# codyd51/gypsum

Measured on NVIDIA H100. Metric: IQ Msamples/s through 32-PRN x 41-Doppler acquisition (1 ms non-coherent, 2.046 Msps complex64), higher is better.
Workload: dtype f32

## Files before the change

gypsum_b200/csrc/engine.cu:

```cuda
#include <algorithm>
#include <cstddef>
#include <cstdio>
#include <cstdlib>
#include <cstring>
#include <map>
#include <numeric>
#include <string>
#include <tuple>
#include <utility>
#include <vector>

#include "../../include/gypsum_b200.h"
#include "bits_core.cuh"
#include "kernels.cuh"
#include "fix_core.cuh"
#include "nav_core.cuh"
#include "orbit_core.cuh"

using namespace gb;

static_assert(sizeof(gb200_cell_record) == sizeof(CellRecord), "ABI record and device record must match");

namespace {

thread_local std::string g_create_error;

struct DeviceMemory {
    static cudaError_t alloc(void** p, size_t bytes) { return cudaMalloc(p, bytes); }
    static void free(void* p) { cudaFree(p); }
};
struct PinnedMemory {
    static cudaError_t alloc(void** p, size_t bytes) { return cudaMallocHost(p, bytes); }
    static void free(void* p) { cudaFreeHost(p); }
};

template <class T, class Memory>
struct Buf {
    T* p = nullptr;
    size_t cap = 0;
    Buf() = default;
    Buf(const Buf&) = delete;
    Buf& operator=(const Buf&) = delete;
    Buf(Buf&& o) noexcept : p(std::exchange(o.p, nullptr)), cap(std::exchange(o.cap, 0)) {}
    ~Buf() { release(); }
    cudaError_t ensure(size_t n) {
        if (n <= cap) return cudaSuccess;
        release();
        size_t want = std::max(n, static_cast<size_t>(16));
        cudaError_t e = Memory::alloc(reinterpret_cast<void**>(&p), want * sizeof(T));
        if (e == cudaSuccess) cap = want;
        return e;
    }
    void release() {
        if (p) Memory::free(p);
        p = nullptr;
        cap = 0;
    }
};
template <class T>
using DevBuf = Buf<T, DeviceMemory>;
template <class T>
using PinnedBuf = Buf<T, PinnedMemory>;

constexpr int kL2WindowMb = 16;

int env_int(const char* name, int dflt) {
    const char* v = getenv(name);
    return (v && *v) ? atoi(v) : dflt;
}

}

struct gb200_engine {
    int device = 0, fs = 0, N = 0, s = 0, num_sms = 132;
    cudaStream_t own_stream = nullptr, stream = nullptr;
    DevBuf<float2> tw1, tw2, crep, iq_own, spec, d_replica;
    DevBuf<uint8_t> chips;
    DevBuf<double> d_doppler;
    DevBuf<int> d_ints;
    DevBuf<CellRecord> d_records;
    DevBuf<float> d_profile;
    DevBuf<RefineState> r_state;
    DevBuf<double> r_doppler;
    DevBuf<CellRecord> r_records;
    DevBuf<int> r_ints;
    DevBuf<RefineResult> r_results;
    DevBuf<int> r_cell_prn;
    PinnedBuf<int> rh_cell_prn;
    PinnedBuf<int> rh_ints;
    PinnedBuf<RefineResult> rh_results;
    PinnedBuf<float2> h_iq, h_replica;
    PinnedBuf<CellRecord> h_records;
    PinnedBuf<int> h_ints;
    PinnedBuf<double> h_doubles;
    PinnedBuf<float> h_profile;
    std::vector<double> doppler_cache;
    std::vector<int> prn_cache;
    bool grid_cache_valid = false;
    int n_prn = 0;
    const float2* iq = nullptr;
    int64_t iq_samples = 0;
    int64_t launches = 0;
    size_t spec_budget_bytes = 512u << 20;
    bool timing = false;
    int fused = -1;
    bool fused_configured = false;
    DevBuf<BestRecord> d_best;
    PinnedBuf<BestRecord> h_best;
    struct HostGraph {
        struct Key {
            int n_blocks = 0, M = 0, P = 0, D = 0, kind = 0;
            std::vector<double> dop;
            std::vector<int> prn;
            const void *iq_dev = nullptr, *rec_dev = nullptr, *iq_stage = nullptr, *rec_stage = nullptr, *spec = nullptr;
            const void *d_dop = nullptr, *d_prn = nullptr, *crep = nullptr;
            const void* rec_target = nullptr;
            cudaStream_t stream = nullptr;
            auto ids() const {
                return std::tie(n_blocks, M, P, D, kind, iq_dev, rec_dev, iq_stage, rec_stage, spec, d_dop, d_prn, crep, rec_target,
                                stream);
            }
            bool operator==(const Key& o) const {
                return ids() == o.ids() && dop.size() == o.dop.size() && prn == o.prn &&
                       memcmp(dop.data(), o.dop.data(), sizeof(double) * dop.size()) == 0;
            }
        } key;
        cudaGraphExec_t exec = nullptr;
        int seen = 0;
    } hg;
    std::vector<std::pair<cudaEvent_t, cudaEvent_t>> ev[2];
    size_t ev_used[2] = {0, 0};
    std::string err;

    ~gb200_engine() {
        if (hg.exec) cudaGraphExecDestroy(hg.exec);
        for (auto& pool : ev)
            for (auto& pr : pool) {
                cudaEventDestroy(pr.first);
                cudaEventDestroy(pr.second);
            }
        if (own_stream) cudaStreamDestroy(own_stream);
    }
};

struct TrackerChain {
    struct Output {
        std::vector<int> counts;
        int stride = 0;
        int n_ms = 0;
        bool pending = false;
    };
    Output records;
    Output bits;
// ... 181 lines not shown
        if (stop) cudaEventRecord(stop, e->stream);
    }
};

int pick_rsplit(const gb200_engine* e, int slots, long long n_cells) {
    if (n_cells >= 8LL * e->num_sms * slots) return 1;
    return std::gcd(e->s, slots);
}

size_t unit_floats2(const gb200_engine* e, int M) { return static_cast<size_t>(M) * e->s * 2 * kFft; }

int run_spectra(gb200_engine* e, const float2* iq, int M, const double* dop, int n_doppler, int n_units) {
    SpectraArgs sa{};
    sa.iq = iq;
    sa.doppler = dop;
    sa.spec = e->spec.p;
    sa.tw1 = e->tw1.p;
    sa.tw2 = e->tw2.p;
    sa.block_stride = static_cast<long long>(M) * e->N;
    sa.inv_fs = 1.0 / static_cast<double>(e->fs);
    sa.N = e->N;
    sa.s = e->s;
    sa.M = M;
    sa.n_doppler = n_doppler;
    sa.n_units = n_units;
    GB_LAUNCH(e, 0, launch_doppler_spectra(sa, e->stream));
    return GB200_OK;
}

CorrelateArgs correlate_args(const gb200_engine* e, int M, int kind, int rsplit, CellRecord* records, float* profile) {
    CorrelateArgs ca{};
    ca.spec = e->spec.p;
    ca.crep = e->crep.p;
    ca.tw1 = e->tw1.p;
    ca.tw2 = e->tw2.p;
    ca.records = records;
    ca.profile = profile;
    ca.N = e->N;
    ca.s = e->s;
    ca.M = M;
    ca.kind = kind;
    ca.rsplit = rsplit;
    return ca;
}

int fused_args(gb200_engine* e, int M, FusedArgs* fa) {
    if (!e->fused_configured) {
        GB_CUDA(e, configure_fused_kernel());
        e->fused_configured = true;
    }
    *fa = FusedArgs{};
    fa->iq = e->iq;
    fa->crep = e->crep.p;
    fa->tw1 = e->tw1.p;
    fa->tw2 = e->tw2.p;
    fa->inv_fs = 1.0 / static_cast<double>(e->fs);
    fa->N = e->N;
    fa->M = M;
    return GB200_OK;
}

struct ListPlan {
    std::vector<int> cell_u, cell_out, grp_first, grp_count, grp_prn;
    size_t size() const { return 2 * cell_u.size() + 3 * grp_prn.size(); }
    void write(int* host) const {
        for (const auto* v : {&cell_u, &cell_out, &grp_first, &grp_count, &grp_prn}) host = std::copy(v->begin(), v->end(), host);
// ... 365 lines not shown
    if ((ce = e->tw2.ensure(kFft)) != cudaSuccess) return fail(ce, "cudaMalloc");
    if ((ce = launch_init_tables(e->tw1.p, e->tw2.p, e->stream)) != cudaSuccess) return fail(ce, "init_tables");
    e->launches++;
    if ((ce = cudaStreamSynchronize(e->stream)) != cudaSuccess) return fail(ce, "init_tables sync");
    *out = e;
    return GB200_OK;
}

int gb200_destroy(gb200_engine* e) {
    if (!e) return GB200_OK;
    cudaSetDevice(e->device);
    cudaStreamSynchronize(e->stream);
    delete e;
    return GB200_OK;
}

int gb200_set_stream(gb200_engine* e, void* st) {
    if (!e) return GB200_EINVAL;
    GB_CUDA(e, cudaSetDevice(e->device));
    GB_CUDA(e, cudaStreamSynchronize(e->stream));
    e->stream = st ? static_cast<cudaStream_t>(st) : e->own_stream;
    return GB200_OK;
}

int gb200_set_replicas(gb200_engine* e, const uint8_t* chips, int n_prn) {
    if (!e) return GB200_EINVAL;
    if (!chips || n_prn < 1) GB_FAIL(e, GB200_EINVAL, "need at least one PRN code");
    for (int i = 0; i < n_prn * kChips; ++i)
        if (chips[i] > 1) GB_FAIL(e, GB200_EINVAL, "chips must be 0 or 1");
    GB_CUDA(e, cudaSetDevice(e->device));
    GB_CUDA(e, cudaStreamSynchronize(e->stream));
    GB_CUDA(e, e->chips.ensure(static_cast<size_t>(n_prn) * kChips));
    GB_CUDA(e, e->crep.ensure(static_cast<size_t>(n_prn) * 2 * kFft));
    GB_CUDA(e, cudaMemcpyAsync(e->chips.p, chips, static_cast<size_t>(n_prn) * kChips, cudaMemcpyHostToDevice, e->stream));
    GB_LAUNCH(e, -1, launch_replica_spectra(e->chips.p, n_prn, e->crep.p, e->stream));
    GB_CUDA(e, cudaStreamSynchronize(e->stream));
    e->n_prn = n_prn;
    return GB200_OK;
}

int gb200_upload_iq(gb200_engine* e, const float* iq_host, int64_t n_samples) {
    if (!e) return GB200_EINVAL;
    if (!iq_host || n_samples < 0) GB_FAIL(e, GB200_EINVAL, "bad IQ buffer");
    GB_CUDA(e, cudaSetDevice(e->device));
    GB_CUDA(e, e->iq_own.ensure(static_cast<size_t>(std::max<int64_t>(n_samples, 1))));
    const float2* src = reinterpret_cast<const float2*>(iq_host);
    if (!is_pinned(iq_host)) {
        GB_CUDA(e, cudaStreamSynchronize(e->stream));
        GB_CUDA(e, stage_in(e->h_iq, src, static_cast<size_t>(n_samples)));
    }
    GB_CUDA(e, cudaMemcpyAsync(e->iq_own.p, src, static_cast<size_t>(n_samples) * sizeof(float2), cudaMemcpyHostToDevice,
                               e->stream));
    e->iq = e->iq_own.p;
    e->iq_samples = n_samples;
    return GB200_OK;
}

int gb200_bind_iq_device(gb200_engine* e, const void* iq_device, int64_t n_samples) {
    if (!e) return GB200_EINVAL;
    if (!iq_device || n_samples < 0) GB_FAIL(e, GB200_EINVAL, "bad IQ buffer");
    if (reinterpret_cast<uintptr_t>(iq_device) % 16 != 0) GB_FAIL(e, GB200_EINVAL, "IQ buffer must be 16-byte aligned");
    e->iq = static_cast<const float2*>(iq_device);
    e->iq_samples = n_samples;
    return GB200_OK;
}

int gb200_acquire_grid_device(gb200_engine* e, int n_blocks, int M, const int32_t* prn_idx, int P, const double* dop, int D,
                              int kind, void* out_device) {
// ... 45 lines not shown
                            const double* dop, int D, int kind, gb200_cell_record* out_host) {
    if (!e) return GB200_EINVAL;
    if (!iq_host || !out_host) GB_FAIL(e, GB200_EINVAL, "null buffer");
    GB_TRY(check_grid(e, std::min(n_blocks, M), P, D, prn_idx, dop));
    GB_CUDA(e, cudaSetDevice(e->device));
    const size_t n_iq = static_cast<size_t>(n_blocks) * M * e->N, n_rec = static_cast<size_t>(n_blocks) * P * D;
    const size_t spec_bytes = unit_floats2(e, M) * D * sizeof(float2) * n_blocks;
    if (e->timing || spec_bytes > e->spec_budget_bytes) {
        GB_TRY(gb200_upload_iq(e, iq_host, static_cast<int64_t>(n_iq)));
        return gb200_acquire_grid(e, n_blocks, M, prn_idx, P, dop, D, kind, out_host);
    }
    GB_CUDA(e, cudaStreamSynchronize(e->stream));
    GB_CUDA(e, e->iq_own.ensure(n_iq));
    GB_CUDA(e, e->h_iq.ensure(n_iq));
    GB_CUDA(e, e->d_records.ensure(n_rec));
    GB_CUDA(e, e->h_records.ensure(n_rec));
    const float2* h2d_src = reinterpret_cast<const float2*>(iq_host);
    const bool eager_src = n_iq * sizeof(float2) > (64u << 10) && is_pinned(iq_host);
    if (!eager_src) GB_CUDA(e, stage_in(e->h_iq, h2d_src, n_iq));
    e->iq = e->iq_own.p;
    e->iq_samples = static_cast<int64_t>(n_iq);

    GB_TRY(check_replicas(e));
    GB_TRY(check_prns(e, prn_idx, P));
    GB_TRY(upload_grid_axes(e, prn_idx, P, dop, D));
    const bool direct = n_rec * sizeof(CellRecord) <= (256u << 10);
    void* caller_alias = nullptr;
    const bool to_caller = direct && is_pinned(out_host, &caller_alias) && caller_alias;
    CellRecord* rec_target = to_caller ? static_cast<CellRecord*>(caller_alias) : direct ? e->h_records.p : e->d_records.p;
    auto& g = e->hg;
    auto key = [&] {
        return gb200_engine::HostGraph::Key{n_blocks, M, P, D, kind, {dop, dop + D}, {prn_idx, prn_idx + P},
                                            e->iq_own.p, e->d_records.p, e->h_iq.p, e->h_records.p, e->spec.p,
                                            e->d_doppler.p, e->d_ints.p, e->crep.p, rec_target, e->stream};
    };
    const bool same = g.seen && g.key == key();
    auto enqueue = [&]() -> int {
        GB_CUDA(e, cudaMemcpyAsync(e->iq_own.p, h2d_src, n_iq * sizeof(float2), cudaMemcpyHostToDevice, e->stream));
        GB_TRY(run_grid(e, n_blocks, M, prn_idx, P, dop, D, kind, rec_target));
        if (!direct)
            GB_CUDA(e, cudaMemcpyAsync(e->h_records.p, e->d_records.p, n_rec * sizeof(CellRecord), cudaMemcpyDeviceToHost, e->stream));
        return GB200_OK;
    };
    if (eager_src) {
        GB_TRY(enqueue());
    } else if (same && g.exec) {
        GB_CUDA(e, cudaGraphLaunch(g.exec, e->stream));
        e->launches += 2;
    } else if (same && !g.exec && g.seen == 1) {
        g.seen = 2;
        GB_CUDA(e, cudaStreamBeginCapture(e->stream, cudaStreamCaptureModeThreadLocal));
        int rc = enqueue();
        cudaGraph_t graph = nullptr;
        cudaError_t ce = cudaStreamEndCapture(e->stream, &graph);
        if (rc == GB200_OK && ce == cudaSuccess && graph) ce = cudaGraphInstantiate(&g.exec, graph, 0);
        if (graph) cudaGraphDestroy(graph);
        if (rc != GB200_OK || ce != cudaSuccess || !g.exec) {
            cudaGetLastError();
            g.exec = nullptr;
            GB_TRY(enqueue());
        } else {
            GB_CUDA(e, cudaGraphLaunch(g.exec, e->stream));
        }
    } else {
        if (!same) {
            if (g.exec) cudaGraphExecDestroy(g.exec);
            g.exec = nullptr;
// ... 966 lines not shown
```

gypsum_b200/csrc/kernels.cu:

```cuda
#include "kernels.cuh"
#include "ptx_helpers.cuh"
#include "warp_fft.cuh"

namespace gb {

__global__ void k_init_tables(float2* tw1, float2* tw2) {
    const int t = blockIdx.x * blockDim.x + threadIdx.x;
    if (t >= 1024) return;
    {
        const int k1 = t >> 5, l = t & 31;
        double s, c;
        sincospi(-2.0 * ((l * k1) & 1023) / 1024.0, &s, &c);
        tw1[pidx(k1, l)] = make_float2(static_cast<float>(c), static_cast<float>(s));
    }
    {
        double s, c;
        sincospi(-2.0 * t / 2048.0, &s, &c);
        tw2[zpos(t)] = make_float2(static_cast<float>(c), static_cast<float>(s));
    }
}

__global__ void __launch_bounds__(128) k_replica_spectra(const uint8_t* chips, float2* crep) {
    __shared__ double2 cs[kPad];
    __shared__ uint8_t c[1024];
    const int p = blockIdx.y;
    for (int t = threadIdx.x; t < kPad; t += blockDim.x) {
        double s, co;
        sincospi(2.0 * t / kPad, &s, &co);
        cs[t] = make_double2(co, s);
    }
    for (int t = threadIdx.x; t < kChips; t += blockDim.x) c[t] = chips[p * kChips + t];
    __syncthreads();
    const int g = blockIdx.x * blockDim.x + threadIdx.x;
    double re, im;
    replica_spectrum_bin(c, g, cs, re, im);
    crep[(static_cast<size_t>(p) * 2 + (g & 1)) * kFft + zpos(g >> 1)] = make_float2(static_cast<float>(re), static_cast<float>(im));
}

__host__ __device__ constexpr int spec_warps(int s) { return 2 * s >= 8 ? 8 : 2 * s; }
constexpr int kCarrierTable = 64;

__host__ __device__ constexpr bool spec_alias(int s) { return 2 * s <= 8; }
__host__ __device__ constexpr int spec_f2(int s) {
    return spec_alias(s) ? (s * kFft > spec_warps(s) * kTileF2 ? s * kFft : spec_warps(s) * kTileF2)
                         : s * kFft + spec_warps(s) * kTileF2;
}

template <int S>
__global__ void __launch_bounds__(spec_warps(S) * 32, S == 2 ? 4 : 1) k_doppler_spectra(const SpectraArgs a) {
    constexpr int kSpecWarps = spec_warps(S);
    constexpr int kSpecThreads = kSpecWarps * 32;
    extern __shared__ __align__(16) float2 smem[];
    float2* ypoly = smem;
    float2* tiles = spec_alias(S) ? smem : smem + S * kFft;
    float2* coarse = smem + spec_f2(S);

    const int unit = blockIdx.x / a.M, i = blockIdx.x % a.M;
    const int b = unit / a.n_doppler, d = unit % a.n_doppler;
    const double f = a.doppler[d];
    if (isnan(f)) return;
    const float2* __restrict__ src = a.iq + static_cast<size_t>(b) * a.block_stride + static_cast<size_t>(i) * a.N;
    const int tid = threadIdx.x;

    constexpr int kIter = (kChips * S + kSpecThreads - 1) / kSpecThreads;
    constexpr int kBatch = kIter < 16 ? kIter : 16;
    float2 v[kBatch];
#pragma unroll
    for (int k = 0; k < kBatch; ++k) {
        const int n = tid + k * kSpecThreads;
// ... 210 lines not shown
                    pair_barrier(pair);
                }
                Peak t;
                float fsum;
                thread_peak16(acc, lane, h, a.s, r, t, fsum);
                t.sum = static_cast<double>(fsum);
                peak_merge(pk, t);
                if (PROFILE && KIND != kKindCoherent) {
#pragma unroll
                    for (int jj = 0; jj < 16; ++jj) {
                        const int q = lane + 32 * (16 * h + jj);
                        if (q < kChips) a.profile[a.s * q + r] = acc[jj];
                    }
                }
            }
            warp_reduce_peak(pk);
            if (KIND == kKindCoherent) warp_reduce_probe(pr_re, pr_im);
            if (lane == 0) store_partial(partial + warp, pk, pr_re, pr_im);
        }
        if (a.rsplit == 1) {
            if (active) pair_barrier(pair);
        } else {
            __syncthreads();
        }
        if (active && (pair % a.rsplit) == 0 && h == 0 && lane == 0) {
            float pre, pim;
            const Peak m = merge_partials(partial + warp, 2 * a.rsplit, pre, pim);
            write_record(a.records + out, m, pre, pim);
        }
        if (a.rsplit != 1) __syncthreads();
    }
}

template <int NW, bool SINGLE_MS>
__global__ void __launch_bounds__(NW * 32, 1) k_correlate_w2048(const CorrelateArgs a) {
    extern __shared__ __align__(16) float2 smem[];
    constexpr int kCrepOdd = kFft;
    float2* crep_s = smem;
    float2* tw1_s = crep_s + 2 * kFft;
    float2* tw1o_s = tw1_s + kFft;
    float2* tiles = tw1o_s + kFft / 2;
    PeakPartial* partial = reinterpret_cast<PeakPartial*>(tiles + NW * kTile64F2);
    uint64_t* mbar = reinterpret_cast<uint64_t*>(partial + NW);

    const int warp = threadIdx.x >> 5, lane = threadIdx.x & 31;
    float2* tile = tiles + warp * kTile64F2;

    uint32_t parity = 0;
    if (threadIdx.x == 0) mbar_init(mbar, 1);
    __syncthreads();
    if (threadIdx.x == 0) {
        mbar_expect_tx(mbar, kFft * sizeof(float2));
        bulk_g2s(tw1_s, a.tw1, kFft * sizeof(float2), mbar);
    }
    mbar_wait(mbar, parity);
    parity ^= 1;
    if (warp == 0) w2048_odd_twiddles(lane, tw1_s, tw1o_s);
    __syncthreads();
    asm volatile("griddepcontrol.wait;" ::: "memory");

    const int cells_per_group = NW / a.rsplit;
    const int r_per_warp = a.s / a.rsplit;
    const int my_cell = warp / a.rsplit;
    const int my_r0 = (warp % a.rsplit) * r_per_warp;
    const size_t unit_stride = static_cast<size_t>(a.M) * a.s * 2 * kFft;
    int cur_prn = -1;

    const int wch = (a.grid_mode && a.win_chunks > 0 && a.win_chunks < a.chunks) ? a.win_chunks : a.chunks;
    const int n_win = a.grid_mode ? (a.chunks + wch - 1) / wch : 1;
    for (int w = 0; w < n_win; ++w) {
    const int ch_w = a.grid_mode ? min(wch, a.chunks - w * wch) : 0;
    const int ng_w = a.grid_mode ? a.P * ch_w : a.n_groups;
    const int n_cta = static_cast<int>(gridDim.x);
    const int per_cta = ng_w / n_cta, extra = ng_w - per_cta * n_cta;
    const int extra_full = a.grid_mode ? (a.P * wch) % n_cta : 0;
    const int slot = static_cast<int>((blockIdx.x + n_cta - static_cast<int>((static_cast<long long>(w) * extra_full) % n_cta)) % n_cta);
    int g0 = slot * per_cta + min(slot, extra);
    int g1 = g0 + per_cta + (slot < extra ? 1 : 0);
    if (n_win == 1) {
        g0 = static_cast<int>(static_cast<long long>(blockIdx.x) * ng_w / n_cta);
        g1 = static_cast<int>(static_cast<long long>(blockIdx.x + 1) * ng_w / n_cta);
    }
    int gpl = 0, gch = 0;
    if (a.grid_mode && g0 < g1) {
        gpl = g0 / ch_w;
        gch = g0 - gpl * ch_w;
    }

    for (int g = g0; g < g1; ++g) {
        const GroupCell gc = decode_group(a, g, cells_per_group, my_cell, w * wch, ch_w, gpl, gch);
        const bool active = gc.active;
        const int unit = gc.unit, out = gc.out;
        if (gc.prn != cur_prn) {
            stage_replica(a, gc.prn, crep_s, mbar, parity, (warp >> 2) * a.stag_a + (warp & 3) * a.stag_b);
            cur_prn = gc.prn;
        }

        if (active) {
            Peak pk;
            peak_init(pk);
            const float2* __restrict__ spec_u = a.spec + static_cast<size_t>(unit) * unit_stride;
            for (int r = my_r0; r < my_r0 + r_per_warp; ++r) {
                float acc[32];
#pragma unroll
                for (int k = 0; k < 32; ++k) acc[k] = 0.f;
                const int n_iter = SINGLE_MS ? 1 : a.M;
                for (int it = 0; it < n_iter; ++it) {
                    const float2* __restrict__ p = spec_u + static_cast<size_t>(it * a.s + r) * 2 * kFft;
                    {
                        float2 hx[32];
                        load_mul_vec(hx, lane, p, crep_s);
                        w2048_phase1<0>(hx, lane, tw1_s, tile);
                    }
                    {
                        float2 hx[32];
                        load_mul_vec(hx, lane, p + kFft, crep_s + kFft);
                        w2048_phase1_odd(hx, lane, tw1_s, tw1o_s, tile);
                    }
                    __syncwarp();
                    float2 x[64];
                    w2048_phase2(x, lane, tile);
                    __syncwarp();
#pragma unroll
                    for (int k = 0; k < 32; ++k) {
                        if (SINGLE_MS) acc[k] = gb_mag(x[k]);
                        else acc[k] += gb_mag(x[k]);
                    }
                }
                Peak t;
                float fsum[2];
                thread_peak32(acc, lane, a.s, r, t, fsum);
                t.sum = static_cast<double>(fsum[0]);
                peak_merge(pk, t);
                pk.sum += static_cast<double>(fsum[1]);
            }
            warp_reduce_peak(pk);
            if (lane == 0) {
                if (a.rsplit == 1) write_record(a.records + out, pk, 0.f, 0.f);
                else store_partial(partial + warp, pk, 0.f, 0.f);
            }
        }
        if (a.rsplit != 1) {
            __syncthreads();
            if (active && (warp % a.rsplit) == 0 && lane == 0) {
                float pre, pim;
                write_record(a.records + out, merge_partials(partial + warp, a.rsplit, pre, pim), 0.f, 0.f);
            }
            __syncthreads();
        }
// ... 145 lines not shown
    return cudaGetLastError();
}

cudaError_t launch_refine_init(int n_sv, RefineState* st, cudaStream_t s) {
    k_refine_init<<<(n_sv + 63) / 64, 64, 0, s>>>(n_sv, st);
    return cudaGetLastError();
}
cudaError_t launch_refine_plan(int n_sv, double spread, const RefineState* st, double* doppler, cudaStream_t s) {
    const int n = n_sv * kRefineMaxBins;
    k_refine_plan<<<(n + 127) / 128, 128, 0, s>>>(n_sv, spread, st, doppler);
    return cudaGetLastError();
}
cudaError_t launch_refine_select(int n_sv, int N, const CellRecord* rec, const double* doppler, RefineState* st, cudaStream_t s) {
    k_refine_select<<<(n_sv + 63) / 64, 64, 0, s>>>(n_sv, N, rec, doppler, st);
    return cudaGetLastError();
}
cudaError_t launch_refine_coherent_plan(int n_sv, const RefineState* st, double* doppler, int* probe, cudaStream_t s) {
    k_refine_coherent_plan<<<(n_sv + 63) / 64, 64, 0, s>>>(n_sv, st, doppler, probe);
    return cudaGetLastError();
}
cudaError_t launch_refine_finalize(int n_sv, const RefineState* st, const CellRecord* rec, RefineResult* out, cudaStream_t s) {
    k_refine_finalize<<<(n_sv + 63) / 64, 64, 0, s>>>(n_sv, st, rec, out);
    return cudaGetLastError();
}

size_t spectra_smem_bytes(int s) {
    return (static_cast<size_t>(spec_f2(s)) + kCarrierTable) * sizeof(float2);
}
size_t correlate_smem_bytes() {
    return (4 * static_cast<size_t>(kFft) + 2 * kPairs * kTileF2) * sizeof(float2) + 2 * kPairs * sizeof(PeakPartial) + 16;
}

size_t correlate_w2048_smem_bytes(int nw) {
    return (3 * static_cast<size_t>(kFft) + kFft / 2 + static_cast<size_t>(nw) * kTile64F2) * sizeof(float2) +
           nw * sizeof(PeakPartial) + 16;
}

bool spectra_supports(int s) {
    switch (s) {
#define GB_CASE(S) case S:
        GB_FOR_EACH_RATE(GB_CASE) return true;
#undef GB_CASE
        default: return false;
    }
}

template <int S>
static cudaError_t spectra_attr() {
    return cudaFuncSetAttribute(k_doppler_spectra<S>, cudaFuncAttributeMaxDynamicSharedMemorySize,
                                static_cast<int>(spectra_smem_bytes(S)));
}
cudaError_t configure_kernels() {
    cudaError_t e;
#define GB_ATTR(S) if ((e = spectra_attr<S>()) != cudaSuccess) return e;
    GB_FOR_EACH_RATE(GB_ATTR)
#undef GB_ATTR
    const int sm = static_cast<int>(correlate_smem_bytes());
    if ((e = cudaFuncSetAttribute(k_correlate_cells<kKindCoherent, false>, cudaFuncAttributeMaxDynamicSharedMemorySize, sm))) return e;
    if ((e = cudaFuncSetAttribute(k_correlate_cells<kKindCoherent, true>, cudaFuncAttributeMaxDynamicSharedMemorySize, sm))) return e;
    if ((e = cudaFuncSetAttribute(k_correlate_cells<kKindNonCoherent, true>, cudaFuncAttributeMaxDynamicSharedMemorySize, sm))) return e;
    if ((e = cudaFuncSetAttribute(k_correlate_w2048<12, true>, cudaFuncAttributeMaxDynamicSharedMemorySize,
                                  static_cast<int>(correlate_w2048_smem_bytes(12)))) != cudaSuccess)
        return e;
    return cudaFuncSetAttribute(k_correlate_w2048<8, false>, cudaFuncAttributeMaxDynamicSharedMemorySize,
                                static_cast<int>(correlate_w2048_smem_bytes(8)));
}

cudaError_t launch_init_tables(float2* tw1, float2* tw2, cudaStream_t st) {
    k_init_tables<<<4, 256, 0, st>>>(tw1, tw2);
    return cudaGetLastError();
}
cudaError_t launch_replica_spectra(const uint8_t* chips_dev, int n_prn, float2* crep, cudaStream_t st) {
    k_replica_spectra<<<dim3(kPad / 128, n_prn), 128, 0, st>>>(chips_dev, crep);
    return cudaGetLastError();
}
cudaError_t launch_doppler_spectra(const SpectraArgs& a, cudaStream_t st) {
    const int grid = a.n_units * a.M;
    const size_t sm = spectra_smem_bytes(a.s);
    switch (a.s) {
#define GB_CASE(S) case S: k_doppler_spectra<S><<<grid, spec_warps(S) * 32, sm, st>>>(a); break;
        GB_FOR_EACH_RATE(GB_CASE)
#undef GB_CASE
        default: return cudaErrorInvalidValue;
    }
    return cudaGetLastError();
}

constexpr int kW2048StaggerRowNs = 600, kW2048StaggerColNs = 150;

static bool pair_kernel(int kind, bool profile) { return kind == kKindCoherent || profile; }

int correlate_slots(int kind, int M, bool profile) {
    if (pair_kernel(kind, profile)) return kPairs;
    return M == 1 ? 12 : 8;
}

template <class K>
static void launch_dependent(K kernel, const CorrelateArgs& a, int grid, int block, size_t sm, cudaStream_t st) {
    cudaLaunchConfig_t cfg{};
    cfg.gridDim = dim3(grid);
    cfg.blockDim = dim3(block);
    cfg.dynamicSmemBytes = sm;
    cfg.stream = st;
    cudaLaunchAttribute attr[1];
    attr[0].id = cudaLaunchAttributeProgrammaticStreamSerialization;
    attr[0].val.programmaticStreamSerializationAllowed = 1;
    cfg.attrs = attr;
    cfg.numAttrs = 1;
    cudaLaunchKernelEx(&cfg, kernel, a);
}

cudaError_t launch_correlate(const CorrelateArgs& a0, int grid, cudaStream_t st) {
    if (pair_kernel(a0.kind, a0.profile != nullptr)) {
        const size_t sm = correlate_smem_bytes();
        if (a0.kind != kKindCoherent) k_correlate_cells<kKindNonCoherent, true><<<grid, kPairs * 64, sm, st>>>(a0);
        else if (a0.profile) k_correlate_cells<kKindCoherent, true><<<grid, kPairs * 64, sm, st>>>(a0);
        else k_correlate_cells<kKindCoherent, false><<<grid, kPairs * 64, sm, st>>>(a0);
        return cudaGetLastError();
    }
    CorrelateArgs a = a0;
    a.stag_a = kW2048StaggerRowNs;
    a.stag_b = kW2048StaggerColNs;
    if (a.M == 1) launch_dependent(k_correlate_w2048<12, true>, a, grid, 12 * 32, correlate_w2048_smem_bytes(12), st);
    else launch_dependent(k_correlate_w2048<8, false>, a, grid, 8 * 32, correlate_w2048_smem_bytes(8), st);
    return cudaGetLastError();
}

}
```

gypsum_b200/csrc/kernels.cuh:

```cuda
#pragma once
#include "gb_common.cuh"
#include "tracker_core.cuh"

namespace gb {

constexpr int kKindCoherent = 1;
constexpr int kKindNonCoherent = 2;

struct SpectraArgs {
    const float2* iq;
    const double* doppler;
    float2* spec;
    const float2* tw1;
    const float2* tw2;
    long long block_stride;
    double inv_fs;
    int N, s, M, n_doppler, n_units;
};

struct CorrelateArgs {
    const float2* spec;
    const float2* crep;
    const float2* tw1;
    const float2* tw2;
    CellRecord* records;
    float* profile;
    int N, s, M, kind;
    int rsplit;
    int n_groups;
    int grid_mode, P, D, n_blocks, chunks;
    int win_chunks;
    const int* prn_idx;
    const int* grp_first;
    const int* grp_count;
    const int* grp_prn;
    const int* cell_u;
    const int* cell_out;
    const int* cell_probe;
    int stag_a, stag_b;
    const double* cell_gate;
};

constexpr int kRefineMaxBins = 32;
struct RefineState {
    double center;
    double kept_doppler;
    double kept_strength;
    int kept_index;
    int have_kept;
};
struct RefineResult {
    double doppler;
    double strength;
    float probe_re, probe_im;
    int code_phase;
    int pad_;
};
struct BestRecord {
    double doppler;
    double strength;
    float peak;
    int code_phase;
    int bin;
    int pad_;
};
cudaError_t launch_best_bins(int n_rows, int D, int N, const CellRecord* rec, const double* doppler, BestRecord* out,
                             cudaStream_t s);
cudaError_t launch_refine_plan(int n_sv, double spread, const RefineState* st, double* doppler, cudaStream_t s);
cudaError_t launch_refine_select(int n_sv, int N, const CellRecord* rec, const double* doppler, RefineState* st, cudaStream_t s);
cudaError_t launch_refine_coherent_plan(int n_sv, const RefineState* st, double* doppler, int* probe, cudaStream_t s);
cudaError_t launch_refine_finalize(int n_sv, const RefineState* st, const CellRecord* rec, RefineResult* out, cudaStream_t s);
cudaError_t launch_refine_init(int n_sv, RefineState* st, cudaStream_t s);
// ... 74 lines not shown
    double* reset;
    int* prev;
    double* slide1;
    FixRecord* out;
    int n_channels, n_ms;
    int solver;
};
cudaError_t launch_position_fixes(const FixArgs& a, cudaStream_t st);

struct FusedArgs {
    const float2* iq;
    const double* doppler;
    const int* prn;
    const int* probe;
    CellRecord* records;
    const float2* crep;
    const float2* tw1;
    const float2* tw2;
    double inv_fs;
    int N, M, n_cells;
};
bool fused_supports(int s);
cudaError_t configure_fused_kernel();
cudaError_t launch_acquire_fused(const FusedArgs& a, int s, int kind, cudaStream_t st);

size_t track_smem_bytes(int N, int s);
cudaError_t configure_track_kernel();
cudaError_t launch_track_channels(const TrackArgs& a, cudaStream_t st);
cudaError_t launch_integrate_bits(const BitArgs& a, cudaStream_t st);
cudaError_t launch_decode_subframes(const NavArgs& a, cudaStream_t st);
size_t spectra_smem_bytes(int s);
bool spectra_supports(int s);
cudaError_t launch_init_tables(float2* tw1, float2* tw2, cudaStream_t st);
cudaError_t launch_replica_spectra(const uint8_t* chips_dev, int n_prn, float2* crep, cudaStream_t st);
cudaError_t launch_doppler_spectra(const SpectraArgs& a, cudaStream_t st);
int correlate_slots(int kind, int M, bool profile);
cudaError_t launch_correlate(const CorrelateArgs& a, int grid, cudaStream_t st);
cudaError_t launch_correlate_generic(const float2* iq, const float2* replica, int N, int n_ms, double doppler, double inv_fs,
                                     int kind, float* out, cudaStream_t st);
cudaError_t configure_kernels();

}
```

gypsum_b200/csrc/ptx_helpers.cuh:

```cuda
#pragma once
#include <stdint.h>

#include "gb_common.cuh"

namespace gb {

__device__ __forceinline__ uint32_t smem_u32(const void* p) { return static_cast<uint32_t>(__cvta_generic_to_shared(p)); }
__device__ __forceinline__ void mbar_init(uint64_t* bar, int count) {
    asm volatile("mbarrier.init.shared::cta.b64 [%0], %1;" ::"r"(smem_u32(bar)), "r"(count));
    asm volatile("fence.mbarrier_init.release.cluster;" ::: "memory");
}
__device__ __forceinline__ void mbar_expect_tx(uint64_t* bar, uint32_t bytes) {
    asm volatile("mbarrier.arrive.expect_tx.shared::cta.b64 _, [%0], %1;" ::"r"(smem_u32(bar)), "r"(bytes) : "memory");
}
__device__ __forceinline__ void bulk_g2s(void* dst, const void* src, uint32_t bytes, uint64_t* bar) {
    asm volatile("cp.async.bulk.shared::cluster.global.mbarrier::complete_tx::bytes [%0], [%1], %2, [%3];" ::"r"(
                     smem_u32(dst)),
                 "l"(src), "r"(bytes), "r"(smem_u32(bar))
                 : "memory");
}
__device__ __forceinline__ void mbar_wait(uint64_t* bar, uint32_t parity) {
    asm volatile(
        "{\n"
        ".reg .pred p;\n"
        "WAIT_%=:\n"
        "mbarrier.try_wait.parity.shared::cta.b64 p, [%0], %1;\n"
        "@p bra DONE_%=;\n"
        "bra WAIT_%=;\n"
        "DONE_%=:\n"
        "}\n" ::"r"(smem_u32(bar)),
        "r"(parity)
        : "memory");
}
__device__ __forceinline__ void pair_barrier(int pair) { asm volatile("bar.sync %0, 64;" ::"r"(pair + 1) : "memory"); }


__device__ __forceinline__ void cp_async16(void* dst, const void* src) {
    asm volatile("cp.async.cg.shared.global [%0], [%1], 16;" ::"r"(smem_u32(dst)), "l"(src) : "memory");
}
__device__ __forceinline__ void cp_async8(void* dst, const void* src) {
    asm volatile("cp.async.ca.shared.global [%0], [%1], 8;" ::"r"(smem_u32(dst)), "l"(src) : "memory");
}
__device__ __forceinline__ void prefetch_l2_bulk(const void* src, uint32_t bytes) {
    asm volatile("cp.async.bulk.prefetch.L2.global [%0], %1;" ::"l"(src), "r"(bytes) : "memory");
}
__device__ __forceinline__ void cp_async_commit() { asm volatile("cp.async.commit_group;" ::: "memory"); }
template <int N>
__device__ __forceinline__ void cp_async_wait() {
    asm volatile("cp.async.wait_group %0;" ::"n"(N) : "memory");
}

__device__ __forceinline__ void warp_reduce_peak(Peak& p) {
// ... 19 lines not shown
```

gypsum_b200/csrc/warp_fft.cuh:

```cuda
#pragma once
#include "cplx2.cuh"
#include "fft32_gen.cuh"
#include "gb_common.cuh"

namespace gb {


GB_HD GB_INLINE int pidx(int j, int lane) { return (((j >> 1) * 32 + lane) << 1) | (j & 1); }
GB_HD GB_INLINE int zpos(int m) { return pidx(m >> 5, m & 31); }

GB_HD GB_INLINE void ld_pair(const float2* p, float2& a, float2& b) {
#if defined(__CUDA_ARCH__)
    const float4 v = *reinterpret_cast<const float4*>(p);
    a = make_float2(v.x, v.y);
    b = make_float2(v.z, v.w);
#else
    a = p[0];
    b = p[1];
#endif
}
GB_HD GB_INLINE void st_pair(float2* p, float2 a, float2 b) {
#if defined(__CUDA_ARCH__)
    *reinterpret_cast<float4*>(p) = make_float4(a.x, a.y, b.x, b.y);
#else
// ... 197 lines not shown
    const int first = __ffs(eq) - 1, c = __popc(eq);
#else
    const int first = eq ? __builtin_ctz(eq) : -1, c = __builtin_popcount(eq);
#endif
    out.mx = m;
    out.idx = s * (lane + 32 * first) + r;
    out.cnt = c;
    out.sum = 0.0;
    fsum[0] = s0;
    fsum[1] = s1;
}

}

namespace gb {

GB_HD GB_INLINE int padded_chip(const uint8_t* chips, int m) {
    if (m < kChips) return chips[m] ? 1 : -1;
    if (m >= kPad - (kChips - 1)) return chips[m - (kPad - kChips)] ? 1 : -1;
    return 0;
}

GB_HD GB_INLINE void replica_spectrum_bin(const uint8_t* chips, int g, const double2* cs, double& re, double& im) {
    double ar = 0.0, ai = 0.0;
    for (int m = 0; m < kPad; ++m) {
        const int c = padded_chip(chips, m);
        if (c == 0) continue;
        const double2 w = cs[(g * m) & (kPad - 1)];
        ar += c * w.x;
        ai += c * w.y;
    }
    re = ar / kPad;
    im = ai / kPad;
}

}

namespace gb {

constexpr int kT64Stride = 33;
constexpr int kTile64F2 = 64 * kT64Stride;

#define GB_W2048_TABLE                                                                                                  \
    {1.000000000e+00f, 0.000000000e+00f}, {9.999952938e-01f, -3.067956763e-03f}, {9.999811753e-01f, -6.135884649e-03f},  \
    {9.999576446e-01f, -9.203754782e-03f}, {9.999247018e-01f, -1.227153829e-02f}, {9.998823475e-01f, -1.533920628e-02f}, \
    {9.998305818e-01f, -1.840672991e-02f}, {9.997694054e-01f, -2.147408028e-02f}, {9.996988187e-01f, -2.454122852e-02f}, \
    {9.996188225e-01f, -2.760814578e-02f}, {9.995294175e-01f, -3.067480318e-02f}, {9.994306046e-01f, -3.374117185e-02f}, \
    {9.993223846e-01f, -3.680722294e-02f}, {9.992047586e-01f, -3.987292759e-02f}, {9.990777278e-01f, -4.293825693e-02f}, \
    {9.989412932e-01f, -4.600318213e-02f}, {9.987954562e-01f, -4.906767433e-02f}, {9.986402182e-01f, -5.213170468e-02f}, \
    {9.984755806e-01f, -5.519524435e-02f}, {9.983015449e-01f, -5.825826450e-02f}, {9.981181129e-01f, -6.132073630e-02f}, \
    {9.979252862e-01f, -6.438263093e-02f}, {9.977230666e-01f, -6.744391956e-02f}, {9.975114561e-01f, -7.050457339e-02f}, \
    {9.972904567e-01f, -7.356456360e-02f}, {9.970600703e-01f, -7.662386139e-02f}, {9.968202993e-01f, -7.968243797e-02f}, \
    {9.965711458e-01f, -8.274026455e-02f}, {9.963126122e-01f, -8.579731234e-02f}, {9.960447009e-01f, -8.885355258e-02f}, \
    {9.957674145e-01f, -9.190895650e-02f}, {9.954807555e-01f, -9.496349533e-02f}

template <int H>
GB_HD GB_INLINE void w2048_phase1(float2 (&x)[32], int lane, const float2* tw1, float2* tile) {
    constexpr float kW[32][2] = {GB_W2048_TABLE};
    fft32_inv(x);
    float2* row = tile + (H * 32 + lane) * kT64Stride;
#pragma unroll
    for (int kp = 0; kp < 16; ++kp) {
        float2 w0, w1;
        ld_pair(tw1 + 2 * (kp * 32 + lane), w0, w1);
#pragma unroll
        for (int q = 0; q < 2; ++q) {
// ... 45 lines not shown
```

Baseline: 188.6.

## Store half replica spectrum via conjugate symmetry, double-buffer PRN staging with mbarriers

The replica spectrum is real-signal derived, so only half is stored; the other half is reconstructed by conjugation in a new load_mul_vec_half. The correlate kernel now keeps two half-size replica buffers in shared memory, using full/empty mbarrier pairs and an atomic election so one lane stages the next PRN while other warps still use the current one. This replaces the previous staggered synchronous staging and its timing constants. It cuts shared-memory footprint and global traffic for the replica, but adds mbarrier and atomic coordination whose correctness depends on all warps advancing PRNs in lockstep.

```diff
diff --git a/gypsum_b200/csrc/engine.cu b/gypsum_b200/csrc/engine.cu
--- a/gypsum_b200/csrc/engine.cu
+++ b/gypsum_b200/csrc/engine.cu
@@ -16,6 +16,7 @@
 #include "fix_core.cuh"
 #include "nav_core.cuh"
 #include "orbit_core.cuh"
+#include "warp_fft.cuh"
 
 using namespace gb;
 
@@ -74,7 +75,7 @@
 struct gb200_engine {
     int device = 0, fs = 0, N = 0, s = 0, num_sms = 132;
     cudaStream_t own_stream = nullptr, stream = nullptr;
-    DevBuf<float2> tw1, tw2, crep, iq_own, spec, d_replica;
+    DevBuf<float2> tw1, tw2, crep, crep_half, iq_own, spec, d_replica;
     DevBuf<uint8_t> chips;
     DevBuf<double> d_doppler;
     DevBuf<int> d_ints;
@@ -113,12 +114,12 @@
             std::vector<double> dop;
             std::vector<int> prn;
             const void *iq_dev = nullptr, *rec_dev = nullptr, *iq_stage = nullptr, *rec_stage = nullptr, *spec = nullptr;
-            const void *d_dop = nullptr, *d_prn = nullptr, *crep = nullptr;
+            const void *d_dop = nullptr, *d_prn = nullptr, *crep = nullptr, *crep_half = nullptr;
             const void* rec_target = nullptr;
             cudaStream_t stream = nullptr;
             auto ids() const {
-                return std::tie(n_blocks, M, P, D, kind, iq_dev, rec_dev, iq_stage, rec_stage, spec, d_dop, d_prn, crep, rec_target,
-                                stream);
+                return std::tie(n_blocks, M, P, D, kind, iq_dev, rec_dev, iq_stage, rec_stage, spec, d_dop, d_prn, crep, crep_half,
+                                rec_target, stream);
             }
             bool operator==(const Key& o) const {
                 return ids() == o.ids() && dop.size() == o.dop.size() && prn == o.prn &&
@@ -366,6 +367,7 @@
     CorrelateArgs ca{};
     ca.spec = e->spec.p;
     ca.crep = e->crep.p;
+    ca.crep_half = e->crep_half.p;
     ca.tw1 = e->tw1.p;
     ca.tw2 = e->tw2.p;
     ca.records = records;
@@ -797,8 +799,9 @@
     GB_CUDA(e, cudaStreamSynchronize(e->stream));
     GB_CUDA(e, e->chips.ensure(static_cast<size_t>(n_prn) * kChips));
     GB_CUDA(e, e->crep.ensure(static_cast<size_t>(n_prn) * 2 * kFft));
+    GB_CUDA(e, e->crep_half.ensure(static_cast<size_t>(n_prn) * kCrepHalf));
     GB_CUDA(e, cudaMemcpyAsync(e->chips.p, chips, static_cast<size_t>(n_prn) * kChips, cudaMemcpyHostToDevice, e->stream));
-    GB_LAUNCH(e, -1, launch_replica_spectra(e->chips.p, n_prn, e->crep.p, e->stream));
+    GB_LAUNCH(e, -1, launch_replica_spectra(e->chips.p, n_prn, e->crep.p, e->crep_half.p, e->stream));
     GB_CUDA(e, cudaStreamSynchronize(e->stream));
     e->n_prn = n_prn;
     return GB200_OK;
@@ -910,7 +913,7 @@
     auto key = [&] {
         return gb200_engine::HostGraph::Key{n_blocks, M, P, D, kind, {dop, dop + D}, {prn_idx, prn_idx + P},
                                             e->iq_own.p, e->d_records.p, e->h_iq.p, e->h_records.p, e->spec.p,
-                                            e->d_doppler.p, e->d_ints.p, e->crep.p, rec_target, e->stream};
+                                            e->d_doppler.p, e->d_ints.p, e->crep.p, e->crep_half.p, rec_target, e->stream};
     };
     const bool same = g.seen && g.key == key();
     auto enqueue = [&]() -> int {
diff --git a/gypsum_b200/csrc/kernels.cu b/gypsum_b200/csrc/kernels.cu
--- a/gypsum_b200/csrc/kernels.cu
+++ b/gypsum_b200/csrc/kernels.cu
@@ -20,7 +20,7 @@
     }
 }
 
-__global__ void __launch_bounds__(128) k_replica_spectra(const uint8_t* chips, float2* crep) {
+__global__ void __launch_bounds__(128) k_replica_spectra(const uint8_t* chips, float2* crep, float2* crep_half) {
     __shared__ double2 cs[kPad];
     __shared__ uint8_t c[1024];
     const int p = blockIdx.y;
@@ -34,7 +34,13 @@
     const int g = blockIdx.x * blockDim.x + threadIdx.x;
     double re, im;
     replica_spectrum_bin(c, g, cs, re, im);
-    crep[(static_cast<size_t>(p) * 2 + (g & 1)) * kFft + zpos(g >> 1)] = make_float2(static_cast<float>(re), static_cast<float>(im));
+    const float2 v = make_float2(static_cast<float>(re), static_cast<float>(im));
+    crep[(static_cast<size_t>(p) * 2 + (g & 1)) * kFft + zpos(g >> 1)] = v;
+    int pos, conj_pos;
+    crep_half_pos(g & 1, g >> 1, &pos, &conj_pos);
+    float2* half = crep_half + static_cast<size_t>(p) * kCrepHalf;
+    if (pos >= 0) half[pos] = v;
+    if (conj_pos >= 0) half[conj_pos] = make_float2(v.x, -v.y);
 }
 
 __host__ __device__ constexpr int spec_warps(int s) { return 2 * s >= 8 ? 8 : 2 * s; }
@@ -311,29 +317,41 @@
     }
 }
 
+__device__ __forceinline__ void stage_replica_half(const CorrelateArgs& a, int prn, float2* dst, uint64_t* full) {
+    mbar_expect_tx(full, kCrepHalf * sizeof(float2));
+    bulk_g2s(dst, a.crep_half + static_cast<size_t>(prn) * kCrepHalf, kCrepHalf * sizeof(float2), full);
+}
+
 template <int NW, bool SINGLE_MS>
 __global__ void __launch_bounds__(NW * 32, 1) k_correlate_w2048(const CorrelateArgs a) {
     extern __shared__ __align__(16) float2 smem[];
-    constexpr int kCrepOdd = kFft;
     float2* crep_s = smem;
-    float2* tw1_s = crep_s + 2 * kFft;
+    float2* tw1_s = crep_s + 2 * kCrepHalf;
     float2* tw1o_s = tw1_s + kFft;
     float2* tiles = tw1o_s + kFft / 2;
     PeakPartial* partial = reinterpret_cast<PeakPartial*>(tiles + NW * kTile64F2);
     uint64_t* mbar = reinterpret_cast<uint64_t*>(partial + NW);
+    uint64_t* full = mbar + 1;
+    uint64_t* empty = mbar + 3;
+    int* staged = reinterpret_cast<int*>(mbar + 5);
 
     const int warp = threadIdx.x >> 5, lane = threadIdx.x & 31;
     float2* tile = tiles + warp * kTile64F2;
 
-    uint32_t parity = 0;
-    if (threadIdx.x == 0) mbar_init(mbar, 1);
+    if (threadIdx.x == 0) {
+        mbar_init(mbar, 1);
+        mbar_init(full, 1);
+        mbar_init(full + 1, 1);
+        mbar_init(empty, NW);
+        mbar_init(empty + 1, NW);
+        *staged = 0;
+    }
     __syncthreads();
     if (threadIdx.x == 0) {
         mbar_expect_tx(mbar, kFft * sizeof(float2));
         bulk_g2s(tw1_s, a.tw1, kFft * sizeof(float2), mbar);
     }
-    mbar_wait(mbar, parity);
-    parity ^= 1;
+    mbar_wait(mbar, 0);
     if (warp == 0) w2048_odd_twiddles(lane, tw1_s, tw1o_s);
     __syncthreads();
     asm volatile("griddepcontrol.wait;" ::: "memory");
@@ -343,7 +361,8 @@
     const int my_cell = warp / a.rsplit;
     const int my_r0 = (warp % a.rsplit) * r_per_warp;
     const size_t unit_stride = static_cast<size_t>(a.M) * a.s * 2 * kFft;
-    int cur_prn = -1;
+    int cur_prn = -1, k = 0;
+    const float2* crep_w = crep_s;
 
     const int wch = (a.grid_mode && a.win_chunks > 0 && a.win_chunks < a.chunks) ? a.win_chunks : a.chunks;
     const int n_win = a.grid_mode ? (a.chunks + wch - 1) / wch : 1;
@@ -371,8 +390,18 @@
         const bool active = gc.active;
         const int unit = gc.unit, out = gc.out;
         if (gc.prn != cur_prn) {
-            stage_replica(a, gc.prn, crep_s, mbar, parity, (warp >> 2) * a.stag_a + (warp & 3) * a.stag_b);
+            __syncwarp();
+            if (lane == 0) {
+                if (k > 0) mbar_arrive(empty + ((k - 1) & 1));
+                if (atomicCAS(staged, k, k + 1) == k) {
+                    if (k >= 2) mbar_wait(empty + (k & 1), ((k - 2) >> 1) & 1);
+                    stage_replica_half(a, gc.prn, crep_s + (k & 1) * kCrepHalf, full + (k & 1));
+                }
+            }
+            mbar_wait(full + (k & 1), (k >> 1) & 1);
+            crep_w = crep_s + (k & 1) * kCrepHalf;
             cur_prn = gc.prn;
+            ++k;
         }
 
         if (active) {
@@ -388,12 +417,12 @@
                     const float2* __restrict__ p = spec_u + static_cast<size_t>(it * a.s + r) * 2 * kFft;
                     {
                         float2 hx[32];
-                        load_mul_vec(hx, lane, p, crep_s);
+                        load_mul_vec_half<0>(hx, lane, p, crep_w);
                         w2048_phase1<0>(hx, lane, tw1_s, tile);
                     }
                     {
                         float2 hx[32];
-                        load_mul_vec(hx, lane, p + kFft, crep_s + kFft);
+                        load_mul_vec_half<1>(hx, lane, p + kFft, crep_w + kCrepHalfOdd);
                         w2048_phase1_odd(hx, lane, tw1_s, tw1o_s, tile);
                     }
                     __syncwarp();
@@ -605,8 +634,8 @@
 }
 
 size_t correlate_w2048_smem_bytes(int nw) {
-    return (3 * static_cast<size_t>(kFft) + kFft / 2 + static_cast<size_t>(nw) * kTile64F2) * sizeof(float2) +
-           nw * sizeof(PeakPartial) + 16;
+    return (2 * static_cast<size_t>(kCrepHalf) + kFft + kFft / 2 + static_cast<size_t>(nw) * kTile64F2) * sizeof(float2) +
+           nw * sizeof(PeakPartial) + 6 * sizeof(uint64_t);
 }
 
 bool spectra_supports(int s) {
@@ -643,8 +672,8 @@
     k_init_tables<<<4, 256, 0, st>>>(tw1, tw2);
     return cudaGetLastError();
 }
-cudaError_t launch_replica_spectra(const uint8_t* chips_dev, int n_prn, float2* crep, cudaStream_t st) {
-    k_replica_spectra<<<dim3(kPad / 128, n_prn), 128, 0, st>>>(chips_dev, crep);
+cudaError_t launch_replica_spectra(const uint8_t* chips_dev, int n_prn, float2* crep, float2* crep_half, cudaStream_t st) {
+    k_replica_spectra<<<dim3(kPad / 128, n_prn), 128, 0, st>>>(chips_dev, crep, crep_half);
     return cudaGetLastError();
 }
 cudaError_t launch_doppler_spectra(const SpectraArgs& a, cudaStream_t st) {
@@ -658,8 +687,6 @@
     }
     return cudaGetLastError();
 }
-
-constexpr int kW2048StaggerRowNs = 600, kW2048StaggerColNs = 150;
 
 static bool pair_kernel(int kind, bool profile) { return kind == kKindCoherent || profile; }
 
@@ -683,17 +710,14 @@
     cudaLaunchKernelEx(&cfg, kernel, a);
 }
 
-cudaError_t launch_correlate(const CorrelateArgs& a0, int grid, cudaStream_t st) {
-    if (pair_kernel(a0.kind, a0.profile != nullptr)) {
+cudaError_t launch_correlate(const CorrelateArgs& a, int grid, cudaStream_t st) {
+    if (pair_kernel(a.kind, a.profile != nullptr)) {
         const size_t sm = correlate_smem_bytes();
-        if (a0.kind != kKindCoherent) k_correlate_cells<kKindNonCoherent, true><<<grid, kPairs * 64, sm, st>>>(a0);
-        else if (a0.profile) k_correlate_cells<kKindCoherent, true><<<grid, kPairs * 64, sm, st>>>(a0);
-        else k_correlate_cells<kKindCoherent, false><<<grid, kPairs * 64, sm, st>>>(a0);
+        if (a.kind != kKindCoherent) k_correlate_cells<kKindNonCoherent, true><<<grid, kPairs * 64, sm, st>>>(a);
+        else if (a.profile) k_correlate_cells<kKindCoherent, true><<<grid, kPairs * 64, sm, st>>>(a);
+        else k_correlate_cells<kKindCoherent, false><<<grid, kPairs * 64, sm, st>>>(a);
         return cudaGetLastError();
     }
-    CorrelateArgs a = a0;
-    a.stag_a = kW2048StaggerRowNs;
-    a.stag_b = kW2048StaggerColNs;
     if (a.M == 1) launch_dependent(k_correlate_w2048<12, true>, a, grid, 12 * 32, correlate_w2048_smem_bytes(12), st);
     else launch_dependent(k_correlate_w2048<8, false>, a, grid, 8 * 32, correlate_w2048_smem_bytes(8), st);
     return cudaGetLastError();
diff --git a/gypsum_b200/csrc/kernels.cuh b/gypsum_b200/csrc/kernels.cuh
--- a/gypsum_b200/csrc/kernels.cuh
+++ b/gypsum_b200/csrc/kernels.cuh
@@ -21,6 +21,7 @@
 struct CorrelateArgs {
     const float2* spec;
     const float2* crep;
+    const float2* crep_half;
     const float2* tw1;
     const float2* tw2;
     CellRecord* records;
@@ -37,7 +38,6 @@
     const int* cell_u;
     const int* cell_out;
     const int* cell_probe;
-    int stag_a, stag_b;
     const double* cell_gate;
 };
 
@@ -178,7 +178,7 @@
 size_t spectra_smem_bytes(int s);
 bool spectra_supports(int s);
 cudaError_t launch_init_tables(float2* tw1, float2* tw2, cudaStream_t st);
-cudaError_t launch_replica_spectra(const uint8_t* chips_dev, int n_prn, float2* crep, cudaStream_t st);
+cudaError_t launch_replica_spectra(const uint8_t* chips_dev, int n_prn, float2* crep, float2* crep_half, cudaStream_t st);
 cudaError_t launch_doppler_spectra(const SpectraArgs& a, cudaStream_t st);
 int correlate_slots(int kind, int M, bool profile);
 cudaError_t launch_correlate(const CorrelateArgs& a, int grid, cudaStream_t st);
diff --git a/gypsum_b200/csrc/ptx_helpers.cuh b/gypsum_b200/csrc/ptx_helpers.cuh
--- a/gypsum_b200/csrc/ptx_helpers.cuh
+++ b/gypsum_b200/csrc/ptx_helpers.cuh
@@ -18,6 +18,9 @@
                      smem_u32(dst)),
                  "l"(src), "r"(bytes), "r"(smem_u32(bar))
                  : "memory");
+}
+__device__ __forceinline__ void mbar_arrive(uint64_t* bar) {
+    asm volatile("mbarrier.arrive.shared::cta.b64 _, [%0];" ::"r"(smem_u32(bar)) : "memory");
 }
 __device__ __forceinline__ void mbar_wait(uint64_t* bar, uint32_t parity) {
     asm volatile(
diff --git a/gypsum_b200/csrc/warp_fft.cuh b/gypsum_b200/csrc/warp_fft.cuh
--- a/gypsum_b200/csrc/warp_fft.cuh
+++ b/gypsum_b200/csrc/warp_fft.cuh
@@ -253,6 +253,38 @@
     }
     re = ar / kPad;
     im = ai / kPad;
+}
+
+constexpr int kHalfEvenRow = 33;
+constexpr int kCrepHalfOdd = 2 * 8 * kHalfEvenRow;
+constexpr int kCrepHalf = kCrepHalfOdd + kFft / 2;
+
+GB_HD GB_INLINE void crep_half_pos(int h, int i, int* pos, int* conj_pos) {
+    *pos = *conj_pos = -1;
+    const int j = i >> 5, lane = i & 31;
+    if (i < 512) *pos = h ? kCrepHalfOdd + zpos(i) : 2 * ((j >> 1) * kHalfEvenRow + lane) + (j & 1);
+    else if (h == 0 && lane == 0) *conj_pos = 2 * ((15 - (j >> 1)) * kHalfEvenRow + 32) + 1 - (j & 1);
+}
+
+template <int H>
+GB_HD GB_INLINE void load_mul_vec_half(float2 (&x)[32], int lane, const float2* a, const float2* w) {
+    constexpr int kRow = H ? 32 : kHalfEvenRow;
+    const float2* wd = w + 2 * lane;
+    const float2* wm = w + 2 * ((H ? 31 : 32) - lane);
+#pragma unroll
+    for (int jp = 0; jp < 16; ++jp) {
+        float2 a0, a1, w0, w1;
+        ld_pair(a + 2 * (jp * 32 + lane), a0, a1);
+        if (jp < 8) {
+            ld_pair(wd + 2 * jp * kRow, w0, w1);
+            x[2 * jp] = cmul(a0, w0);
+            x[2 * jp + 1] = cmul(a1, w1);
+        } else {
+            ld_pair(wm + 2 * (15 - jp) * kRow, w0, w1);
+            x[2 * jp] = cmulc(a0, w1);
+            x[2 * jp + 1] = cmulc(a1, w0);
+        }
+    }
 }
 
 }
```

Result: faster. 191.1 (median of 6 runs) (+1.3%).
